# facebookresearch/pytorch3d

Hardware: NVIDIA H100
Metric: rasterize frames/sec (fwd+bwd) 512^2 K=8 (higher is better)
Workload: dtype f32

## Files before the change

### pytorch3d_b200/csrc/raster_meshes.cu

```cuda
#include <cfloat>
#include <climits>

#include "binning.cuh"
#include "bulk_copy.cuh"
#include "common.cuh"
#include "raster_math.cuh"

namespace b200r {

constexpr int SETUP_FACES = 256;
#ifndef B200R_MESH_TILE_H
#define B200R_MESH_TILE_H 16
#endif
constexpr int FTW = 16, FTH = B200R_MESH_TILE_H, FTHREADS = FTW * FTH;
static_assert(FTH == 16 || FTH == 8, "16x16 or 16x8 tiles");
constexpr int CHUNK = FTHREADS;
constexpr int SMEMQ_MAX_K = 32;

__device__ __forceinline__ bool face_is_drawable(const Face& f, bool cull_backfaces) {
  const float zmax = fmaxf(fmaxf(f.z0, f.z1), f.z2), zmin = fminf(fminf(f.z0, f.z1), f.z2);
  if (!(zmax >= 0.0f)) return false;
  if ((double)zmin < kEps) return false;
  const float area = edge_fn(f.x0, f.y0, f.x1, f.y1, f.x2, f.y2);
  if (cull_backfaces && area < 0.0f) return false;
// ... 228 lines not shown
    }
#pragma unroll
    for (int r = 0; r < KMAX; ++r) {
      if (r >= n) break;
#pragma unroll
      for (int i = r & 1; i + 1 < KMAX; i += 2) {
        if (i + 1 < n) {
          const bool sw = key_less(z[i + 1], id[i + 1], z[i], id[i]);
          const float za = z[i], zb = z[i + 1];
          z[i] = sw ? zb : za;
          z[i + 1] = sw ? za : zb;
          const int ia = id[i], ib = id[i + 1];
          id[i] = sw ? ib : ia;
          id[i + 1] = sw ? ia : ib;
          const int sa = slot[i], sb = slot[i + 1];
          slot[i] = sw ? sb : sa;
          slot[i + 1] = sw ? sa : sb;
        }
      }
    }
  }
};

template <int KMAX>
struct RegQueue {
  TopK<KMAX> q;
  float4* pay;
  int K;
  __device__ __forceinline__ void reset() { q.init(); }
  __device__ __forceinline__ bool full() const { return q.size >= K; }
  __device__ __forceinline__ float max_z() const { return q.max_z; }
  __device__ __forceinline__ void offer(const Hit& h, int f) { q.offer(h, f, K, pay); }
  __device__ __forceinline__ bool offer_neighbor(const Hit& h, int f, int nb) { return q.offer_neighbor(h, f, nb, pay); }
};

template <bool NB>
struct SmemQueue {
  float* qz;
  int* qi;
  float* qd;
  int K, size, max_idx;
  float max_zv;
  __device__ __forceinline__ void init(unsigned char* base, int K_, int tid) {
    K = K_;
    qz = reinterpret_cast<float*>(base) + tid;
    qi = reinterpret_cast<int*>(base) + K_ * FTHREADS + tid;
    qd = NB ? reinterpret_cast<float*>(base) + 2 * K_ * FTHREADS + tid : nullptr;
    reset();
  }
  __device__ __forceinline__ void reset() {
    size = 0;
    max_idx = -1;
    max_zv = -1000.0f;
  }
  __device__ __forceinline__ bool full() const { return size >= K; }
  __device__ __forceinline__ float max_z() const { return max_zv; }
  __device__ __forceinline__ void put(int slot, const Hit& h, int f) {
    qz[slot * FTHREADS] = h.z;
    qi[slot * FTHREADS] = f;
    if (NB) qd[slot * FTHREADS] = h.dist;
  }
  __device__ __forceinline__ void offer(const Hit& h, int f) {
    if (size < K) {
      put(size, h, f);
      if (h.z > max_zv) {
        max_zv = h.z;
        max_idx = size;
      }
      ++size;
    } else if (h.z < max_zv) {
      const float evicted = max_zv;
      put(max_idx, h, f);
      max_zv = h.z;
      for (int i = 0; i < K; ++i) {
        const float v = qz[i * FTHREADS];
        if (v > max_zv) {
          max_zv = v;
          max_idx = i;
        }
      }
      if (max_zv == evicted) flag_tie();
    } else if (h.z == max_zv) {
      flag_tie();
    }
  }
  __device__ __forceinline__ bool offer_neighbor(const Hit& h, int f, int nb) {
    int at = -1;
    for (int i = 0; i < size; ++i)
      if (qi[i * FTHREADS] == nb) {
        at = i;
        break;
      }
    if (at < 0) return false;
    if (NB && fabsf(h.dist) < fabsf(qd[at * FTHREADS])) {
      put(at, h, f);
      if (h.z > max_zv) {
        max_zv = h.z;
        max_idx = at;
      }
    }
    return true;
  }
  __device__ __forceinline__ void sort() {
    for (int i = 1; i < size; ++i) {
      const float tz = qz[i * FTHREADS];
      const int ti = qi[i * FTHREADS];
      int j = i - 1;
      while (j >= 0 && key_less(tz, ti, qz[j * FTHREADS], qi[j * FTHREADS])) {
        qz[(j + 1) * FTHREADS] = qz[j * FTHREADS];
        qi[(j + 1) * FTHREADS] = qi[j * FTHREADS];
        --j;
      }
      qz[(j + 1) * FTHREADS] = tz;
      qi[(j + 1) * FTHREADS] = ti;
    }
  }
};

struct __align__(16) FaceChunk {
  float4 box[CHUNK];
  float4 a[CHUNK];
  float4 b[CHUNK];
  float4 c[CHUNK];
};

__device__ __forceinline__ void stage_face(FaceChunk& s, int slot, const float* __restrict__ face_verts,
                                           const int64_t* __restrict__ neighbor, int f, float sqrt_blur,
                                           bool cull_backfaces) {
  const float* v = face_verts + (int64_t)f * 9;
  const Face fc = {__ldg(v + 0), __ldg(v + 1), __ldg(v + 2), __ldg(v + 3), __ldg(v + 4),
                   __ldg(v + 5), __ldg(v + 6), __ldg(v + 7), __ldg(v + 8)};
  float xmin = FLT_MAX, xmax = -FLT_MAX, ymin = FLT_MAX, ymax = -FLT_MAX;
  if (face_is_drawable(fc, cull_backfaces)) face_box(fc, sqrt_blur, xmin, xmax, ymin, ymax);
  s.box[slot] = make_float4(xmin, xmax, ymin, ymax);
  s.a[slot] = make_float4(fc.x0, fc.y0, fc.x1, fc.y1);
  s.b[slot] = make_float4(fc.x2, fc.y2, bary_denominator(fc), __int_as_float(f));
  const int nb = neighbor ? (int)__ldg(neighbor + f) : -1;
  s.c[slot] = make_float4(fc.z0, fc.z1, fc.z2, __int_as_float(nb));
}

template <typename T>
__device__ __forceinline__ void out_store(T* ptr, const T v) {
  __stcs(ptr, v);
}

struct FineParams {
  const float* face_verts;
  const int64_t* neighbor;
  const float4* rec;
  const int64_t* first;
  const int64_t* num;
  const int* tile_offset;
  const int* tile_order;
  int* pairs;
  int64_t capacity;
  int n0;
  int N, H, W, K, TY, TX;
  float rx, ry, blur_radius, sqrt_blur;
  int persp, clip, cull;
  int smem_ints;
  int64_t* pix_to_face;
  float* zbuf;
  float* bary;
  float* dists;
};

__device__ __forceinline__ void thread_pixel(int tile_x, int tile_y, int& xo, int& yo) {
  const int lane = threadIdx.x & 31, w = threadIdx.x >> 5;
  xo = tile_x * TILE + (w & 1) * 8 + (lane & 7);
  yo = tile_y * TILE + (w >> 1) * 4 + (lane >> 3);
}
__device__ __forceinline__ void fthread_pixel(int tile_x, int tile_y, int& xo, int& yo) {
  const int lane = threadIdx.x & 31, w = threadIdx.x >> 5;
  xo = tile_x * FTW + (w & 1) * 8 + (lane & 7);
  yo = tile_y * FTH + (w >> 1) * 4 + (lane >> 3);
}

__device__ __forceinline__ float warp_min(float v) {
#pragma unroll
  for (int d = 16; d > 0; d >>= 1) v = fminf(v, __shfl_xor_sync(0xffffffffu, v, d));
  return v;
}
__device__ __forceinline__ float warp_max(float v) {
#pragma unroll
  for (int d = 16; d > 0; d >>= 1) v = fmaxf(v, __shfl_xor_sync(0xffffffffu, v, d));
  return v;
}

constexpr int ROUND = 64;

struct FineStage {
  float4 a[CHUNK];
  float4 b[CHUNK];
  float4 c[CHUNK];
  union {
    float4 box[CHUNK];
    unsigned mask[CHUNK / 32][FTHREADS];
    int sort_buf[2 * FTHREADS];
    unsigned long long sort_buf64[2 * FTHREADS];
  } u;
  unsigned rng[CHUNK];
  float col[FTW], row[FTH];
  int tie;
  unsigned char tie_lane[FTHREADS];
};

__device__ __forceinline__ void flag_tie() {
#ifndef B200R_EXP_NOWATCH
  extern __shared__ __align__(16) unsigned char smem_raw[];
  reinterpret_cast<FineStage*>(smem_raw)->tie = 1;
  reinterpret_cast<FineStage*>(smem_raw)->tie_lane[threadIdx.x] = 1;
#endif
}

template <int P>
__device__ __forceinline__ void store_pair_run(float4* run, const float4 (&mine)[P], int odd, bool vA, bool vB) {
  constexpr int H = P / 2;
  constexpr int CE = (P + 1) / 2;
  float4 recv[H > 0 ? H : 1];
#pragma unroll
  for (int r = 0; r < H; ++r) {
    const float4 send = odd ? mine[2 * (CE + r) - P] : mine[2 * r + 1];
    recv[r].x = __shfl_xor_sync(0xffffffffu, send.x, 1);
    recv[r].y = __shfl_xor_sync(0xffffffffu, send.y, 1);
    recv[r].z = __shfl_xor_sync(0xffffffffu, send.z, 1);
    recv[r].w = __shfl_xor_sync(0xffffffffu, send.w, 1);
  }
#pragma unroll
  for (int j = 0; j < P; ++j) {
    const float4 ve = 2 * j < P ? mine[2 * j < P ? 2 * j : 0] : recv[j >= CE ? j - CE : 0];
    const float4 vo = 2 * j + 1 < P ? recv[2 * j + 1 < P ? j : 0] : mine[2 * j + 1 >= P ? 2 * j + 1 - P : 0];
    const bool target_a = odd ? (2 * j + 1 < P) : (2 * j < P);
    if (target_a ? vA : vB) out_store(run + 2 * j + odd, odd ? vo : ve);
  }
}

template <int P>
__device__ __forceinline__ void store_pair_split(float4* runA, float4* runB, const float4 (&mine)[P], int odd,
                                                 bool vA, bool vB) {
  static_assert(P % 2 == 0, "an even number of 16-byte pieces per run");
  float4 recv[P / 2];
#pragma unroll
  for (int r = 0; r < P / 2; ++r) {
    const float4 send = odd ? mine[2 * r] : mine[2 * r + 1];
    recv[r].x = __shfl_xor_sync(0xffffffffu, send.x, 1);
    recv[r].y = __shfl_xor_sync(0xffffffffu, send.y, 1);
    recv[r].z = __shfl_xor_sync(0xffffffffu, send.z, 1);
    recv[r].w = __shfl_xor_sync(0xffffffffu, send.w, 1);
  }
#pragma unroll
  for (int r = 0; r < P / 2; ++r)
    if (vA) out_store(runA + 2 * r + odd, odd ? recv[r] : mine[2 * r]);
#pragma unroll
  for (int r = 0; r < P / 2; ++r)
    if (vB) out_store(runB + 2 * r + odd, odd ? mine[2 * r + 1] : recv[r]);
}

template <int KMAX>
__device__ __forceinline__ void write_empty_tile(const FineParams& p, int n, int tile_x, int tile_y) {
  const int tid = threadIdx.x;
  const int x0 = tile_x * FTW, y0 = tile_y * FTH;
  const int K = p.K;
  if ((KMAX == 0 || K == KMAX) && (K % 4) == 0 && x0 + FTW <= p.W && y0 + FTH <= p.H) {
    const float4 m1 = make_float4(-1.f, -1.f, -1.f, -1.f);
    const int KK = KMAX > 0 ? KMAX : K;
    const int SEG_I = FTW * KK / 2;
    const int SEG_F = FTW * KK / 4;
#pragma unroll
    for (int e = tid; e < FTH * SEG_I; e += FTHREADS) {
      const int64_t o = (((int64_t)n * p.H + y0 + e / SEG_I) * p.W + x0) * KK;
      out_store(reinterpret_cast<longlong2*>(p.pix_to_face + o) + e % SEG_I, make_longlong2(-1ll, -1ll));
    }
#pragma unroll
    for (int e = tid; e < FTH * SEG_F; e += FTHREADS) {
      const int64_t o = (((int64_t)n * p.H + y0 + e / SEG_F) * p.W + x0) * KK;
      out_store(reinterpret_cast<float4*>(p.zbuf + o) + e % SEG_F, m1);
      out_store(reinterpret_cast<float4*>(p.dists + o) + e % SEG_F, m1);
    }
#pragma unroll
    for (int e = tid; e < FTH * SEG_F * 3; e += FTHREADS) {
      const int64_t o = (((int64_t)n * p.H + y0 + e / (SEG_F * 3)) * p.W + x0) * KK;
      out_store(reinterpret_cast<float4*>(p.bary + o * 3) + e % (SEG_F * 3), m1);
    }
    return;
  }
  int xo, yo;
  fthread_pixel(tile_x, tile_y, xo, yo);
  if (xo >= p.W || yo >= p.H) return;
  const int64_t o = (((int64_t)n * p.H + yo) * p.W + xo) * K;
  for (int k = 0; k < K; ++k) {
    p.pix_to_face[o + k] = -1ll;
    p.zbuf[o + k] = -1.0f;
    p.dists[o + k] = -1.0f;
    p.bary[(o + k) * 3 + 0] = -1.0f;
    p.bary[(o + k) * 3 + 1] = -1.0f;
    p.bary[(o + k) * 3 + 2] = -1.0f;
  }
}

template <class Q, bool NB>
__device__ __forceinline__ void consider_face(const FineStage& sh, int j, float px, float py, float blur_radius,
                                              bool persp, bool clip, Q& q) {
  const float4 fa = sh.a[j], fb = sh.b[j], fc = sh.c[j];
  const Face f = {fa.x, fa.y, fc.x, fa.z, fa.w, fc.y, fb.x, fb.y, fc.z};
  const int nb = NB ? __float_as_int(fc.w) : -1;
  Hit h;
// ... 103 lines not shown
#define B200R_SCAN_LANES 4
#endif
      constexpr int SL = B200R_SCAN_LANES;
      const int dr = tid & (SL - 1);
      for (int fslot = tid / SL; fslot < nc; fslot += FTHREADS / SL) {
        const unsigned rg = sh.rng[fslot];
        const int c_lo = rg & 255, c_hi = (rg >> 8) & 255, r_lo = (rg >> 16) & 255, r_hi = rg >> 24;
        if (c_lo > c_hi) continue;
        const float4 fa = sh.a[fslot], fb = sh.b[fslot];
        const bool pos = fb.z > 0.0f;
        unsigned* mrow = sh.u.mask[fslot >> 5];
        const unsigned bit = 1u << (fslot & 31);
        const float dx0 = fsub(fb.x, fa.z), dy0 = fsub(fb.y, fa.w);
        const float dx1 = fsub(fa.x, fb.x), dy1 = fsub(fa.y, fb.y);
        const float dx2 = fsub(fa.z, fa.x), dy2 = fsub(fa.w, fa.y);
        for (int r = r_lo + dr; r <= r_hi; r += SL) {
          const float qy = sh.row[r];
          const float t0 = fmul(fsub(qy, fa.w), dx0), t1 = fmul(fsub(qy, fb.y), dx1), t2 = fmul(fsub(qy, fa.y), dx2);
          unsigned* mpix = mrow + (r >> 2) * 64 + (r & 3) * 8;
          for (int c0 = c_lo; c0 <= c_hi; c0 += 4) {
#pragma unroll
            for (int u = 0; u < 4; ++u) {
              const int c = c0 + u;
              if (c <= c_hi) {
                const float qx = sh.col[c];
                const float e0 = ffma(fsub(qx, fa.z), dy0, -t0);
                const float e1 = ffma(fsub(qx, fb.x), dy1, -t1);
                const float e2 = ffma(fsub(qx, fa.x), dy2, -t2);
                const bool ok = pos ? (e0 > 0.0f && e1 > 0.0f && e2 > 0.0f) : (e0 < 0.0f && e1 < 0.0f && e2 < 0.0f);
                if (ok) atomicOr(mpix + (c >> 3) * 32 + (c & 7), bit);
              }
            }
          }
        }
      }
      __syncthreads();
      const float px = sh.col[lc], py = sh.row[lr];
#ifdef B200R_EXP_OLDWALK
      for (int w = 0; w < nwords; ++w) {
        unsigned m = sh.u.mask[w][tid];
        while (m != 0u) {
          const int j = w * 32 + __ffs((int)m) - 1;
          m &= m - 1u;
          consider_face<Q, NB>(sh, j, px, py, blur_radius, persp, clip, q);
        }
      }
#else
      {
        int w = 0;
        unsigned m = sh.u.mask[0][tid];
        for (;;) {
          while (m == 0u && ++w < nwords) m = sh.u.mask[w][tid];
          if (m == 0u) break;
          const int j = w * 32 + __ffs((int)m) - 1;
          m &= m - 1u;
          consider_face<Q, NB>(sh, j, px, py, blur_radius, persp, clip, q);
        }
      }
#endif
      continue;
    }
    const float px = sh.col[lc], py = sh.row[lr];
    const bool cull_depth = (clip || !persp) && (order == ORDER_DEPTH || count >= 512);
    const float fc0 = sh.col[lc & 8], fc1 = sh.col[(lc & 8) + 7], fr0 = sh.row[lr & 12], fr1 = sh.row[(lr & 12) + 3];
    const float cmin = fminf(fc0, fc1), cmax = fmaxf(fc0, fc1), rmin = fminf(fr0, fr1), rmax = fmaxf(fr0, fr1);
    const bool warp_active = __any_sync(0xffffffffu, valid);
    for (int sub = 0; sub < nc; sub += ROUND) {
      if (!warp_active) break;
      unsigned m0 = 0, m1 = 0;
      {
        const bool h0 = sub + lane < nc, h1 = sub + 32 + lane < nc;
        float4 b0 = make_float4(FLT_MAX, -FLT_MAX, FLT_MAX, -FLT_MAX), b1 = b0;
        if (h0) b0 = sh.u.box[sub + lane];
        if (h1) b1 = sh.u.box[sub + 32 + lane];
        bool keep0 = h0, keep1 = h1;
#ifndef B200R_EXP_NOCULL
        if (cull_depth) {
          const float zcut = warp_max(!valid ? -FLT_MAX : (q.full() ? q.max_z() : FLT_MAX));
          if (zcut < FLT_MAX) {
            const float cx = 0.5f * (cmin + cmax), cy = 0.5f * (rmin + rmax);
            const float hx = 0.5f * (cmax - cmin) * (1.0f + 1e-6f), hy = 0.5f * (rmax - rmin) * (1.0f + 1e-6f);
            if (h0) {
              const float4 fc = sh.c[sub + lane];
              if (!NB || __float_as_int(fc.w) == -1)
                keep0 = !(face_depth_lower_bound(sh.a[sub + lane], sh.b[sub + lane], fc, cx, cy, hx, hy, persp, clip) >
                          zcut);
            }
            if (h1) {
              const float4 fc = sh.c[sub + 32 + lane];
              if (!NB || __float_as_int(fc.w) == -1)
                keep1 = !(face_depth_lower_bound(sh.a[sub + 32 + lane], sh.b[sub + 32 + lane], fc, cx, cy, hx, hy,
                                                 persp, clip) > zcut);
            }
            if (!keep0) b0 = make_float4(FLT_MAX, -FLT_MAX, FLT_MAX, -FLT_MAX);
            if (!keep1) b1 = make_float4(FLT_MAX, -FLT_MAX, FLT_MAX, -FLT_MAX);
            if (!__any_sync(0xffffffffu, keep0 || keep1)) continue;
          }
        }
#endif
        const bool all0 =
            __all_sync(0xffffffffu, !keep0 || (cmin >= b0.x && cmax <= b0.y && rmin >= b0.z && rmax <= b0.w));
        const bool all1 =
            __all_sync(0xffffffffu, !keep1 || (cmin >= b1.x && cmax <= b1.y && rmin >= b1.z && rmax <= b1.w));
        if (all0 && all1) {
          m0 = __ballot_sync(0xffffffffu, keep0);
          m1 = __ballot_sync(0xffffffffu, keep1);
        } else {
          float col[8], row[4];
#pragma unroll
          for (int c = 0; c < 8; ++c) col[c] = sh.col[(lc & 8) + c];
#pragma unroll
          for (int r = 0; r < 4; ++r) row[r] = sh.row[(lr & 12) + r];
          if (keep0) m0 = box_pixel_mask(b0, col, row);
          if (keep1) m1 = box_pixel_mask(b1, col, row);
          m0 = warp_transpose_bits(m0, lane);
          if (sub + 32 < nc) m1 = warp_transpose_bits(m1, lane);
        }
      }
      unsigned long long mine = valid ? (((unsigned long long)m1 << 32) | m0) : 0ull;
      while (__any_sync(0xffffffffu, mine != 0ull)) {
        if (mine != 0ull) {
          const int j = sub + __ffsll((long long)mine) - 1;
          mine &= mine - 1ull;
          consider_face<Q, NB>(sh, j, px, py, blur_radius, persp, clip, q);
        }
      }
    }
  }
}

__device__ __forceinline__ bool tile_saw_tie(const FineStage& sh) {
#ifdef B200R_EXP_NOWATCH
  return false;
#else
  return __syncthreads_or(sh.tie) != 0;
#endif
}

struct TileWork {
  int tile_x, tile_y, n, seg_begin, count;
  bool overflow;
};
__device__ __forceinline__ TileWork tile_work(const FineParams& p) {
  pdl_wait();
  TileWork t;
  int i = ((p.n0 + blockIdx.z) * p.TY + blockIdx.y) * p.TX + blockIdx.x;
  if (p.tile_order != nullptr) {
    i = p.tile_order[i];
    t.tile_x = i % p.TX;
    const int r = i / p.TX;
    t.tile_y = r % p.TY;
    t.n = r / p.TY;
  } else {
    t.tile_x = blockIdx.x;
    t.tile_y = blockIdx.y;
    t.n = p.n0 + blockIdx.z;
  }
  t.seg_begin = p.tile_offset[i];
  const int seg_end = p.tile_offset[i + 1];
  t.overflow = (int64_t)seg_end > p.capacity || seg_end == INT_MAX;
  t.count = t.overflow ? (int)p.num[t.n] : seg_end - t.seg_begin;
  return t;
}

template <bool NB, bool SCAN>
__device__ __forceinline__ int first_walk_order(const FineParams& p, const TileWork& t) {
  if (t.overflow || NB) return ORDER_INDEX;
  if (SCAN) return ORDER_ARRIVAL;
#ifndef B200R_EXP_DEPTHORDER
  return ORDER_INDEX;
#else
  const bool bound = p.clip != 0 || p.persp == 0;
  return (bound && 2 * t.count <= p.smem_ints) ? ORDER_DEPTH : ORDER_INDEX;
#endif
}

#ifndef B200R_FINE_CTAS
#define B200R_FINE_CTAS 4
#endif
#ifndef B200R_FINE_SCAN_CTAS
#define B200R_FINE_SCAN_CTAS 3
#endif
#ifndef B200R_SMEMQ_CTAS
#define B200R_SMEMQ_CTAS 3
#endif
#ifndef B200R_SMEMQ_SCAN_CTAS
#define B200R_SMEMQ_SCAN_CTAS 2
#endif

template <int KMAX, bool NB, bool SCAN>
__global__ void __launch_bounds__(FTHREADS, SCAN ? B200R_FINE_SCAN_CTAS : B200R_FINE_CTAS) mesh_fine_kernel(const FineParams p) {
  extern __shared__ __align__(16) unsigned char smem_raw[];
  FineStage& sh = *reinterpret_cast<FineStage*>(smem_raw);
  const int tid = threadIdx.x, lane = tid & 31;
  const TileWork t = tile_work(p);
  const int tile_x = t.tile_x, tile_y = t.tile_y, n = t.n;
  if (t.count == 0) {
    write_empty_tile<KMAX>(p, n, tile_x, tile_y);
    return;
  }
  int xo, yo;
  fthread_pixel(tile_x, tile_y, xo, yo);
  const bool valid = xo < p.W && yo < p.H;
  const int lc = xo - tile_x * FTW, lr = yo - tile_y * FTH;

  RegQueue<KMAX> rq;
  rq.q.init();
  rq.pay = reinterpret_cast<float4*>(smem_raw + sizeof(FineStage)) + tid;
  rq.K = p.K;
  TopK<KMAX>& q = rq.q;
  float4* pay = rq.pay;
  const int K = p.K;
  int order = first_walk_order<NB, SCAN>(p, t);
  bool active = valid;
  int scratch_ints = p.smem_ints;
  for (;;) {
  fine_tile_body<RegQueue<KMAX>, NB, SCAN>(p, sh, rq, tile_x, tile_y, n, t.seg_begin, t.count, t.overflow, order,
                                           active, scratch_ints, lc, lr);
  if (order == ORDER_DEPTH) {
    if (tile_saw_tie(sh)) {
      active = valid && sh.tie_lane[tid] != 0;
      if (active) rq.reset();
      order = ORDER_INDEX;
      scratch_ints = (int)(sizeof(FineStage) / sizeof(int));
      __syncthreads();
      continue;
    }
  }
  bool stored = false;
  int slot[KMAX];
  q.sort(slot);
  const int64_t o = (((int64_t)n * p.H + yo) * p.W + xo) * K;
  if constexpr ((KMAX % 4) == 0) {
   if (K == KMAX) {
    const int odd = lane & 1;
    const bool vA = __shfl_sync(0xffffffffu, (int)valid, lane & ~1) != 0;
    const bool vB = __shfl_sync(0xffffffffu, (int)valid, lane | 1) != 0;
    const int64_t oa = o - (int64_t)odd * KMAX;
    {
      float4 piece[KMAX / 2];
#pragma unroll
      for (int k = 0; k < KMAX; k += 2) {
        const long long i0 = k >= q.size ? -1ll : (long long)q.id[k];
        const long long i1 = k + 1 >= q.size ? -1ll : (long long)q.id[k + 1];
        piece[k / 2] = make_float4(__int_as_float((int)(i0 & 0xffffffffll)), __int_as_float((int)(i0 >> 32)),
                                   __int_as_float((int)(i1 & 0xffffffffll)), __int_as_float((int)(i1 >> 32)));
      }
      store_pair_run<KMAX / 2>(reinterpret_cast<float4*>(p.pix_to_face + oa), piece, odd, vA, vB);
    }
    {
      float4 piece[KMAX / 4];
#pragma unroll
      for (int k0 = 0; k0 < KMAX; k0 += 4)
        piece[k0 / 4] = make_float4(k0 + 0 >= q.size ? -1.0f : q.z[k0 + 0], k0 + 1 >= q.size ? -1.0f : q.z[k0 + 1],
                                    k0 + 2 >= q.size ? -1.0f : q.z[k0 + 2], k0 + 3 >= q.size ? -1.0f : q.z[k0 + 3]);
      store_pair_run<KMAX / 4>(reinterpret_cast<float4*>(p.zbuf + oa), piece, odd, vA, vB);
    }
    {
      float4 piece[KMAX / 4];
#pragma unroll
      for (int k0 = 0; k0 < KMAX; k0 += 4) {
        float d[4];
#pragma unroll
        for (int u = 0; u < 4; ++u) d[u] = k0 + u >= q.size ? -1.0f : pay[slot[k0 + u] * FTHREADS].x;
        piece[k0 / 4] = make_float4(d[0], d[1], d[2], d[3]);
      }
      store_pair_run<KMAX / 4>(reinterpret_cast<float4*>(p.dists + oa), piece, odd, vA, vB);
    }
    {
      float4 piece[3 * KMAX / 4];
#pragma unroll
      for (int k0 = 0; k0 < KMAX; k0 += 4) {
        float4 w[4];
#pragma unroll
        for (int u = 0; u < 4; ++u)
          w[u] = k0 + u >= q.size ? make_float4(-1.f, -1.f, -1.f, -1.f) : pay[slot[k0 + u] * FTHREADS];
        piece[3 * (k0 / 4) + 0] = make_float4(w[0].y, w[0].z, w[0].w, w[1].y);
        piece[3 * (k0 / 4) + 1] = make_float4(w[1].z, w[1].w, w[2].y, w[2].z);
        piece[3 * (k0 / 4) + 2] = make_float4(w[2].w, w[3].y, w[3].z, w[3].w);
      }
      store_pair_run<3 * KMAX / 4>(reinterpret_cast<float4*>(p.bary + oa * 3), piece, odd, vA, vB);
    }
    stored = true;
   }
  }
  if (!stored && valid) {
#pragma unroll
    for (int k = 0; k < KMAX; ++k) {
      if (k < K) {
        const bool e = k >= q.size;
        const float4 w = e ? make_float4(-1.f, -1.f, -1.f, -1.f) : pay[slot[k] * FTHREADS];
        p.pix_to_face[o + k] = e ? -1ll : (long long)q.id[k];
        p.zbuf[o + k] = e ? -1.0f : q.z[k];
        p.dists[o + k] = w.x;
        p.bary[(o + k) * 3 + 0] = w.y;
        p.bary[(o + k) * 3 + 1] = w.z;
        p.bary[(o + k) * 3 + 2] = w.w;
      }
    }
  }
  if (order != ORDER_ARRIVAL || !tile_saw_tie(sh)) return;
  order = ORDER_INDEX;
  rq.reset();
  }
}

__device__ __forceinline__ void recompute_hit(const FineParams& p, int fi, float px, float py, Hit& h) {
  const float4* r = p.rec + (int64_t)fi * 4;
  const float4 fa = __ldg(r + 0), fb = __ldg(r + 1), fc = __ldg(r + 2);
  const Face f = {fa.x, fa.y, fc.x, fa.z, fa.w, fc.y, fb.x, fb.y, fc.z};
  eval_pixel_face<false>(px, py, f, fb.z, p.blur_radius, p.persp != 0, p.clip != 0, false, 0.0f, h);
}

template <bool NB, bool SCAN>
__global__ void __launch_bounds__(FTHREADS, SCAN ? B200R_SMEMQ_SCAN_CTAS : B200R_SMEMQ_CTAS) mesh_fine_smemq_kernel(const FineParams p) {
  extern __shared__ __align__(16) unsigned char smem_raw[];
  FineStage& sh = *reinterpret_cast<FineStage*>(smem_raw);
  const int tid = threadIdx.x, lane = tid & 31;
  const TileWork t = tile_work(p);
  const int tile_x = t.tile_x, tile_y = t.tile_y, n = t.n;
  if (t.count == 0) {
    write_empty_tile<0>(p, n, tile_x, tile_y);
    return;
  }
  int xo, yo;
  fthread_pixel(tile_x, tile_y, xo, yo);
  const bool valid = xo < p.W && yo < p.H;
  const int lc = xo - tile_x * FTW, lr = yo - tile_y * FTH;
  const int K = p.K;

  SmemQueue<NB> q;
  q.init(smem_raw + sizeof(FineStage), K, tid);
  int order = first_walk_order<NB, SCAN>(p, t);
  bool active = valid;
  int scratch_ints = p.smem_ints;
  for (;;) {
  fine_tile_body<SmemQueue<NB>, NB, SCAN>(p, sh, q, tile_x, tile_y, n, t.seg_begin, t.count, t.overflow, order, active,
                                          scratch_ints, lc, lr);
  if (order == ORDER_DEPTH) {
    if (tile_saw_tie(sh)) {
      active = valid && sh.tie_lane[tid] != 0;
      if (active) q.reset();
      order = ORDER_INDEX;
      scratch_ints = (int)(sizeof(FineStage) / sizeof(int));
      __syncthreads();
      continue;
    }
  }
  q.sort();
  const float px = sh.col[lc], py = sh.row[lr];
  const int64_t o = (((int64_t)n * p.H + yo) * p.W + xo) * K;
  if ((K & 7) == 0) {
    const int odd = lane & 1;
    const bool vA = __shfl_sync(0xffffffffu, (int)valid, lane & ~1) != 0;
    const bool vB = __shfl_sync(0xffffffffu, (int)valid, lane | 1) != 0;
    const int64_t oa = o - (int64_t)odd * K, ob = oa + K;
    for (int g = 0; g < K; g += 8) {
      float4 pi[4], pzv[2], pd[2], pb[6];
      float z[8], d[8], b[24];
      int id[8];
#pragma unroll
      for (int u = 0; u < 8; ++u) {
        Hit h = {-1.0f, -1.0f, -1.0f, -1.0f, -1.0f};
        id[u] = -1;
        if (g + u < q.size) {
          id[u] = q.qi[(g + u) * FTHREADS];
          recompute_hit(p, id[u], px, py, h);
        }
        z[u] = h.z;
        d[u] = h.dist;
        b[3 * u + 0] = h.b0;
        b[3 * u + 1] = h.b1;
        b[3 * u + 2] = h.b2;
      }
#pragma unroll
      for (int u = 0; u < 4; ++u)
        pi[u] = make_float4(__int_as_float(id[2 * u]), __int_as_float(id[2 * u] >> 31),
                            __int_as_float(id[2 * u + 1]), __int_as_float(id[2 * u + 1] >> 31));
#pragma unroll
      for (int u = 0; u < 2; ++u) {
        pzv[u] = make_float4(z[4 * u], z[4 * u + 1], z[4 * u + 2], z[4 * u + 3]);
        pd[u] = make_float4(d[4 * u], d[4 * u + 1], d[4 * u + 2], d[4 * u + 3]);
      }
#pragma unroll
      for (int u = 0; u < 6; ++u) pb[u] = make_float4(b[4 * u], b[4 * u + 1], b[4 * u + 2], b[4 * u + 3]);
      store_pair_split<4>(reinterpret_cast<float4*>(p.pix_to_face + oa + g),
                          reinterpret_cast<float4*>(p.pix_to_face + ob + g), pi, odd, vA, vB);
      store_pair_split<2>(reinterpret_cast<float4*>(p.zbuf + oa + g), reinterpret_cast<float4*>(p.zbuf + ob + g), pzv,
                          odd, vA, vB);
      store_pair_split<2>(reinterpret_cast<float4*>(p.dists + oa + g), reinterpret_cast<float4*>(p.dists + ob + g),
                          pd, odd, vA, vB);
      store_pair_split<6>(reinterpret_cast<float4*>(p.bary + (oa + g) * 3),
                          reinterpret_cast<float4*>(p.bary + (ob + g) * 3), pb, odd, vA, vB);
    }
  } else if (valid) {
  for (int k = 0; k < K; ++k) {
    Hit h = {-1.0f, -1.0f, -1.0f, -1.0f, -1.0f};
    long long id = -1;
    if (k < q.size) {
      const int fi = q.qi[k * FTHREADS];
      recompute_hit(p, fi, px, py, h);
      id = fi;
    }
    p.pix_to_face[o + k] = id;
    p.zbuf[o + k] = h.z;
    p.dists[o + k] = h.dist;
    p.bary[(o + k) * 3 + 0] = h.b0;
    p.bary[(o + k) * 3 + 1] = h.b1;
    p.bary[(o + k) * 3 + 2] = h.b2;
  }
  }
  if (order != ORDER_ARRIVAL || !tile_saw_tie(sh)) return;
  order = ORDER_INDEX;
  q.reset();
  }
}

__global__ void __launch_bounds__(FTHREADS) mesh_fine_bigk_kernel(const FineParams p) {
  __shared__ FaceChunk s;
  const int tid = threadIdx.x, lane = tid & 31;
  const int t = blockIdx.x;
  const int n = t / (p.TY * p.TX);
  const int tile_y = (t / p.TX) % p.TY, tile_x = t % p.TX;
  int xo, yo;
  fthread_pixel(tile_x, tile_y, xo, yo);
  const bool valid = xo < p.W && yo < p.H;
  const float px = pix_to_ndc(p.W - 1 - xo, p.W, p.rx);
  const float py = pix_to_ndc(p.H - 1 - yo, p.H, p.ry);
  const float fx_lo = warp_min(valid ? px : FLT_MAX), fx_hi = warp_max(valid ? px : -FLT_MAX);
  const float fy_lo = warp_min(valid ? py : FLT_MAX), fy_hi = warp_max(valid ? py : -FLT_MAX);
  pdl_wait();
  const int seg_begin = p.tile_offset[t], seg_end = p.tile_offset[t + 1];
  const bool overflow = (int64_t)seg_end > p.capacity || seg_end == INT_MAX;
  const int64_t mesh_first = p.first[n];
  const int count = overflow ? (int)p.num[n] : seg_end - seg_begin;
  const bool persp = p.persp != 0, clip = p.clip != 0, cull = p.cull != 0;
  const int K = p.K;

  if (!overflow && count > 1)
    cta_sort_segment<FTHREADS>(p.pairs + seg_begin, count, reinterpret_cast<int*>(&s),
                               (int)(sizeof(FaceChunk) / sizeof(int)));

  float qz[B200R_MAX_K], qd[B200R_MAX_K];
  int qi[B200R_MAX_K];
  int qn = 0, q_max_idx = -1;
  float q_max_z = -1000.0f;

  for (int base = 0; base < count; base += CHUNK) {
    const int nc = min(CHUNK, count - base);
    __syncthreads();
    if (tid < nc) {
      const int f = overflow ? (int)(mesh_first + base + tid) : p.pairs[seg_begin + base + tid];
      stage_face(s, tid, p.face_verts, p.neighbor, f, p.sqrt_blur, cull);
// ... 131 lines not shown
                                             float (&out)[9]) {
  const float* v = p.face_verts + fi * 9;
  const Face f = {__ldg(v + 0), __ldg(v + 1), __ldg(v + 2), __ldg(v + 3), __ldg(v + 4),
                  __ldg(v + 5), __ldg(v + 6), __ldg(v + 7), __ldg(v + 8)};
  const float den = bary_denominator(f);
  float w0, w1, w2;
  bary_coords(px, py, f, den, w0, w1, w2);
  float c0 = w0, c1 = w1, c2 = w2;
  if (persp) bary_persp(c0, c1, c2, f.z0, f.z1, f.z2);
  float k0 = c0, k1 = c1, k2 = c2;
  if (clip) bary_clip(k0, k1, k2);
  const bool inside = c0 > 0.0f && c1 > 0.0f && c2 > 0.0f;
  const float sgd = inside ? -gd : gd;

  float2 dv0 = make_float2(0.f, 0.f), dv1 = dv0, dv2 = dv0;
  {
    const float e01 = point_line_dist(px, py, f.x0, f.y0, f.x1, f.y1);
    const float e02 = point_line_dist(px, py, f.x0, f.y0, f.x2, f.y2);
    const float e12 = point_line_dist(px, py, f.x1, f.y1, f.x2, f.y2);
    if (e01 <= e02 && e01 <= e12)
      point_line_bwd(px, py, f.x0, f.y0, f.x1, f.y1, sgd, dv0, dv1);
    else if (e02 <= e01 && e02 <= e12)
      point_line_bwd(px, py, f.x0, f.y0, f.x2, f.y2, sgd, dv0, dv2);
    else if (e12 <= e01 && e12 <= e02)
      point_line_bwd(px, py, f.x1, f.y1, f.x2, f.y2, sgd, dv1, dv2);
  }

  float g0 = gb0 + gz * f.z0, g1 = gb1 + gz * f.z1, g2 = gb2 + gz * f.z2;
  if (clip) {
    const float m0 = fmaxf(c0, 0.0f), m1 = fmaxf(c1, 0.0f), m2 = fmaxf(c2, 0.0f);
    float sum = m0 + m1 + m2, gsc = 1.0f;
    if (sum < 1e-5f) {
      gsc = 0.0f;
      sum = 1e-5f;
    }
    const float inv = __frcp_rn(sum), inv2 = gsc * inv * inv;
    const float s0 = -m0 * inv2, s1 = -m1 * inv2, s2 = -m2 * inv2;
    const float cross = g0 * s0 + g1 * s1 + g2 * s2;
    const float n0 = c0 < 0.0f ? 0.0f : g0 * inv + cross;
    const float n1 = c1 < 0.0f ? 0.0f : g1 * inv + cross;
    const float n2 = c2 < 0.0f ? 0.0f : g2 * inv + cross;
    g0 = n0;
    g1 = n1;
    g2 = n2;
  }
  float dz0 = 0.0f, dz1 = 0.0f, dz2 = 0.0f;
  if (persp) {
    const float t0 = w0 * f.z1 * f.z2, t1 = f.z0 * w1 * f.z2, t2 = f.z0 * f.z1 * w2;
    const float dn = fmaxf(t0 + t1 + t2, 1e-8f);
    const float rdn = __frcp_rn(dn);
    const float gdn = (-t0 * g0 - t1 * g1 - t2 * g2) * rdn * rdn;
    const float h0 = gdn + g0 * rdn, h1 = gdn + g1 * rdn, h2 = gdn + g2 * rdn;
    g0 = h0 * f.z1 * f.z2;
    g1 = h1 * f.z0 * f.z2;
    g2 = h2 * f.z0 * f.z1;
    dz0 = h1 * w1 * f.z2 + h2 * w2 * f.z1;
    dz1 = h0 * w0 * f.z2 + h2 * w2 * f.z0;
    dz2 = h0 * w0 * f.z1 + h1 * w1 * f.z0;
  }
  float2 bv0 = make_float2(0.f, 0.f), bv1 = bv0, bv2 = bv0;
  {
    const float rden = __frcp_rn(den);
    const float e0 = edge_fn(px, py, f.x1, f.y1, f.x2, f.y2);
    const float e1 = edge_fn(px, py, f.x2, f.y2, f.x0, f.y0);
    const float e2 = edge_fn(px, py, f.x0, f.y0, f.x1, f.y1);
    float2 dp, da, db, ap, aa, ab;
    const float garea = -(g0 * e0 + g1 * e1 + g2 * e2) * rden * rden;
    edge_bwd(f.x2, f.y2, f.x0, f.y0, f.x1, f.y1, garea, ap, aa, ab);
    bv2.x += ap.x; bv2.y += ap.y;
    bv0.x += aa.x; bv0.y += aa.y;
    bv1.x += ab.x; bv1.y += ab.y;
    edge_bwd(px, py, f.x1, f.y1, f.x2, f.y2, g0 * rden, dp, da, db);
    bv1.x += da.x; bv1.y += da.y;
    bv2.x += db.x; bv2.y += db.y;
    edge_bwd(px, py, f.x2, f.y2, f.x0, f.y0, g1 * rden, dp, da, db);
    bv2.x += da.x; bv2.y += da.y;
    bv0.x += db.x; bv0.y += db.y;
    edge_bwd(px, py, f.x0, f.y0, f.x1, f.y1, g2 * rden, dp, da, db);
    bv0.x += da.x; bv0.y += da.y;
    bv1.x += db.x; bv1.y += db.y;
  }
  out[0] = bv0.x + dv0.x;
  out[1] = bv0.y + dv0.y;
  out[2] = gz * k0 + dz0;
  out[3] = bv1.x + dv1.x;
  out[4] = bv1.y + dv1.y;
  out[5] = gz * k1 + dz1;
  out[6] = bv2.x + dv2.x;
  out[7] = bv2.y + dv2.y;
  out[8] = gz * k2 + dz2;
}

__device__ __forceinline__ void red_add_v2(float* addr, float a, float b) {
  asm volatile("red.global.add.v2.f32 [%0], {%1, %2};" ::"l"(addr), "f"(a), "f"(b) : "memory");
}
__device__ __forceinline__ void warp_scatter(const BackwardParams& p, int face, float (&g)[9], int lane) {
  const unsigned grp = __match_any_sync(0xffffffffu, face);
  const unsigned above = lane == 31 ? 0u : grp & (0xffffffffu << (lane + 1));
  int next = (face >= 0 && above != 0u) ? __ffs((int)above) - 1 : -1;
  while (__any_sync(0xffffffffu, next >= 0)) {
    const int src = next >= 0 ? next : lane;
#pragma unroll
    for (int i = 0; i < 9; ++i) {
      const float v = __shfl_sync(0xffffffffu, g[i], src);
      if (next >= 0) g[i] += v;
    }
    const int nn = __shfl_sync(0xffffffffu, next, src);
    next = next >= 0 ? nn : -1;
  }
  if (face >= 0 && lane == __ffs((int)grp) - 1) {
    if (p.faces != nullptr) {
      const int64_t* fc = p.faces + (int64_t)face * 3;
#pragma unroll
      for (int j = 0; j < 3; ++j) {
        const int64_t vi = __ldg(fc + j);
        if (vi < 0 || vi >= p.V) continue;
        float* o = p.grad_verts + vi * 3;
#ifndef B200R_EXP_BWD_SCALAR_RED
        if (p.g_vec) {
          const bool odd = (vi & 1) != 0;
          const float s1 = odd ? g[3 * j] : g[3 * j + 2];
          const float a = odd ? g[3 * j + 1] : g[3 * j], b = odd ? g[3 * j + 2] : g[3 * j + 1];
          if (s1 != 0.0f) atomicAdd(o + (odd ? 0 : 2), s1);
          if (a != 0.0f || b != 0.0f) red_add_v2(o + (odd ? 1 : 0), a, b);
          continue;
        }
#endif
#pragma unroll
        for (int c = 0; c < 3; ++c)
          if (g[3 * j + c] != 0.0f) atomicAdd(o + c, g[3 * j + c]);
      }
    } else {
      float* o = p.grad_face_verts + (int64_t)face * 9;
#ifndef B200R_EXP_BWD_SCALAR_RED
      if (p.g_vec) {
        const int odd = face & 1;
        atomicAdd(o + (odd ? 0 : 8), odd ? g[0] : g[8]);
#pragma unroll
        for (int j = 0; j < 4; ++j)
          red_add_v2(o + 2 * j + odd, odd ? g[2 * j + 1] : g[2 * j], odd ? g[2 * j + 2] : g[2 * j + 1]);
        return;
      }
#endif
#pragma unroll
      for (int i = 0; i < 9; ++i) atomicAdd(o + i, g[i]);
    }
  }
}

#ifndef B200R_BWD_PF_CTAS
#define B200R_BWD_PF_CTAS 3
#endif
#ifndef B200R_BWD_CTAS
#define B200R_BWD_CTAS 4
#endif
template <int GV, bool PF>
__global__ void __launch_bounds__(TILE_THREADS, PF ? B200R_BWD_PF_CTAS : B200R_BWD_CTAS) mesh_backward_kernel(const BackwardParams p) {
  const int lane = threadIdx.x & 31;
  const int tile_x = blockIdx.x, tile_y = blockIdx.y, n = p.n0 + blockIdx.z;
  int xo, yo;
  thread_pixel(tile_x, tile_y, xo, yo);
  const bool in_image = xo < p.W && yo < p.H;
  const float px = pix_to_ndc(p.W - 1 - xo, p.W, p.rx);
  const float py = pix_to_ndc(p.H - 1 - yo, p.H, p.ry);
  const int K = p.K;
  const int64_t o = in_image ? (((int64_t)n * p.H + yo) * p.W + xo) * K : 0;
  const bool persp = p.persp != 0, clip = p.clip != 0;
  constexpr int G = GV > 0 ? GV : 1;
  static_assert(!PF || GV == 8, "the prefetching variant is the K % 8 == 0 kernel");

  for (int k0 = 0; k0 < K; k0 += G) {
    int fk[G];
    if (GV > 0) {
#pragma unroll
      for (int k = 0; k < G; k += 2) {
        longlong2 v = make_longlong2(-1, -1);
        if (in_image) v = __ldg(reinterpret_cast<const longlong2*>(p.pix_to_face + o + k0 + k));
        fk[k] = (int)v.x;
        fk[k + 1] = (int)v.y;
      }
    } else {
      fk[0] = in_image ? (int)p.pix_to_face[o + k0] : -1;
    }
    float pz[PF ? 4 : 1], pd[PF ? 4 : 1], pb[PF ? 12 : 1];
    if (PF) {
      float4 vz = make_float4(0.f, 0.f, 0.f, 0.f), vd = vz, b0 = vz, b1 = vz, b2 = vz;
      if (fk[0] >= 0) {
        vz = __ldg(reinterpret_cast<const float4*>(p.grad_zbuf + o + k0));
        vd = __ldg(reinterpret_cast<const float4*>(p.grad_dists + o + k0));
        const float4* gb = reinterpret_cast<const float4*>(p.grad_bary + (o + k0) * 3);
        b0 = __ldg(gb + 0);
        b1 = __ldg(gb + 1);
        b2 = __ldg(gb + 2);
      }
      pz[0] = vz.x; pz[1] = vz.y; pz[2] = vz.z; pz[3] = vz.w;
      pd[0] = vd.x; pd[1] = vd.y; pd[2] = vd.z; pd[3] = vd.w;
      pb[0] = b0.x; pb[1] = b0.y; pb[2] = b0.z; pb[3] = b0.w;
      pb[4] = b1.x; pb[5] = b1.y; pb[6] = b1.z; pb[7] = b1.w;
      pb[8] = b2.x; pb[9] = b2.y; pb[10] = b2.z; pb[11] = b2.w;
    }
#pragma unroll 1
    for (int j = 0; j < G; ++j) {
      const int face = fk[0];
#pragma unroll
      for (int u = 0; u + 1 < G; ++u) fk[u] = fk[u + 1];
      float gz = 0.f, gd = 0.f, gb0 = 0.f, gb1 = 0.f, gb2 = 0.f;
      if (PF) {
        gz = pz[0]; gd = pd[0]; gb0 = pb[0]; gb1 = pb[1]; gb2 = pb[2];
#pragma unroll
        for (int u = 0; u < 3; ++u) {
          pz[u] = pz[u + 1];
          pd[u] = pd[u + 1];
        }
#pragma unroll
        for (int u = 0; u < 9; ++u) pb[u] = pb[u + 3];
      }
      if (!__any_sync(0xffffffffu, face >= 0)) continue;
      float g[9] = {0.f, 0.f, 0.f, 0.f, 0.f, 0.f, 0.f, 0.f, 0.f};
      if (face >= 0) {
        const int64_t i = o + k0 + j;
        if (!PF || j >= 4) {
          gz = __ldg(p.grad_zbuf + i);
          gd = __ldg(p.grad_dists + i);
          gb0 = __ldg(p.grad_bary + i * 3);
          gb1 = __ldg(p.grad_bary + i * 3 + 1);
          gb2 = __ldg(p.grad_bary + i * 3 + 2);
        }
        backward_one(p, px, py, face, gz, gd, gb0, gb1, gb2, persp, clip, g);
      }
      warp_scatter(p, face, g, lane);
    }
  }
}

}

__global__ void __launch_bounds__(256) mesh_gather_kernel(const float* __restrict__ verts, int64_t V,
                                                          const int64_t* __restrict__ faces, int64_t F,
                                                          float* __restrict__ face_verts_out) {
  const int64_t e = (int64_t)blockIdx.x * blockDim.x + threadIdx.x;
  if (e >= F * 3) return;
  const int64_t vi = __ldg(faces + e);
  const bool ok = vi >= 0 && vi < V;
#pragma unroll
  for (int c = 0; c < 3; ++c) face_verts_out[e * 3 + c] = ok ? __ldg(verts + vi * 3 + c) : __int_as_float(0x7fc00000);
}

using namespace b200r;

extern "C" size_t b200r_rasterize_meshes_workspace_bytes(int64_t F, int32_t N, int32_t H, int32_t W,
                                                         int64_t pair_capacity) {
  if (F < 0 || N < 0 || H < 0 || W < 0) return 0;
  return carve_workspace(nullptr, F, N, H, W, pair_capacity, FTH, FTW).bytes +
         FACE_RECORD_BYTES * (size_t)(F > 0 ? F : 1);
}

static int forward_impl(const float* face_verts, const float* verts, int64_t V, const int64_t* faces,
                        float* face_verts_out, int64_t F, const int64_t* first, const int64_t* num,
                        const int64_t* neighbor, int32_t N, int32_t H, int32_t W, float blur_radius, int32_t K,
                        int32_t perspective_correct, int32_t clip_barycentric_coords, int32_t cull_backfaces,
                        int64_t* pix_to_face, float* zbuf, float* bary, float* dists, void* workspace,
                        size_t workspace_bytes, int64_t pair_capacity, void* stream_) {
  cudaStream_t stream = static_cast<cudaStream_t>(stream_);
  if (K > B200R_MAX_K) return fail(B200R_ERR_INVALID_ARGUMENT, "Must have points_per_pixel <= 150");
  if (F < 0 || N < 0 || H < 0 || W < 0 || K < 0) return fail(B200R_ERR_INVALID_ARGUMENT, "negative size");
  if (F > INT_MAX) return fail(B200R_ERR_INVALID_ARGUMENT, "more than 2^31-1 packed faces are not supported");
  if ((int64_t)N * H * W * K == 0) return B200R_OK;
  const int TY = div_up(H, FTH), TX = div_up(W, FTW);
  if (TY > 0xFFFE || TX > 0xFFFE) return fail(B200R_ERR_INVALID_ARGUMENT, "image too large");
  const int64_t ntiles = (int64_t)N * TY * TX;
  if (ntiles > INT_MAX) return fail(B200R_ERR_INVALID_ARGUMENT, "too many tiles");
  BinWorkspace ws = carve_workspace(workspace, F, N, H, W, pair_capacity, FTH, FTW);
  const size_t nrec = (size_t)(F > 0 ? F : 1);
  if (workspace == nullptr || workspace_bytes < ws.bytes + FACE_RECORD_BYTES * nrec)
    return fail(B200R_ERR_WORKSPACE, "workspace too small for rasterize_meshes_forward");
  float4* rec = reinterpret_cast<float4*>(static_cast<char*>(workspace) + ws.bytes);

  const float rx = ndc_range(W, H), ry = ndc_range(H, W);
  const float sqrt_blur = sqrtf(blur_radius);

  const bool prof = profiling_enabled();
  if (prof) phase_timer().record(0, stream);
#ifndef B200R_EXP_MEMSET_NODE
  zero_ints_kernel<<<(unsigned)((ntiles + 1023) / 1024), 256, 0, stream>>>(ws.tile_count, ntiles);
  B200R_LAUNCHED("zero_ints_kernel");
#else
  B200R_CUDA_OK(cudaMemsetAsync(ws.tile_count, 0, sizeof(int) * (size_t)ntiles, stream));
#endif
  if (F > 0) {
    const unsigned sgrid = (unsigned)((F + SETUP_FACES - 1) / SETUP_FACES);
#ifndef B200R_EXP_MEMSET_NODE
#define B200R_SETUP_LAUNCH(KERNEL, ...) B200R_CUDA_OK(launch_chained(KERNEL, dim3(sgrid), dim3(SETUP_FACES), 0, stream, __VA_ARGS__))
#else
#define B200R_SETUP_LAUNCH(KERNEL, ...) KERNEL<<<sgrid, SETUP_FACES, 0, stream>>>(__VA_ARGS__)
#endif
    if (faces != nullptr) {
      B200R_SETUP_LAUNCH(mesh_setup_count_kernel<true>, (const float*)nullptr, verts, V, faces, face_verts_out, neighbor, F,
                         first, num, N, H, W, TY, TX, rx, ry, sqrt_blur, cull_backfaces, ws.rect, ws.tile_count, rec);
      face_verts = face_verts_out;
    } else {
      B200R_SETUP_LAUNCH(mesh_setup_count_kernel<false>, face_verts, (const float*)nullptr, (int64_t)0,
                         (const int64_t*)nullptr, (float*)nullptr, neighbor, F, first, num, N, H, W, TY, TX, rx, ry,
                         sqrt_blur, cull_backfaces, ws.rect, ws.tile_count, rec);
    }
#undef B200R_SETUP_LAUNCH
    B200R_LAUNCHED("mesh_setup_count_kernel");
  }
#ifdef B200R_EXP_NOTILEORDER
  int* const tile_order = nullptr;
#else
  int* const tile_order = (blur_radius > 0.0f && ntiles < (1ll << ORDER_BITS)) ? ws.tile_order : nullptr;
#endif
  B200R_CUDA_OK(launch_chained(tile_scan_kernel, dim3(1), dim3(1024), 0, stream, ws.tile_count, ws.tile_offset,
                               (int)ntiles, tile_order));
  B200R_LAUNCHED("tile_scan_kernel");
  if (F > 0) {
    B200R_CUDA_OK(launch_chained(tile_fill_kernel<true>, dim3((unsigned)((F + 255) / 256)), dim3(256), 0, stream,
                                 ws.rect, F, TY, TX, ws.tile_count, ws.pairs, ws.capacity));
    B200R_LAUNCHED("tile_fill_kernel");
  }
  if (prof) phase_timer().record(1, stream);
  FineParams p;
  p.face_verts = face_verts;
  p.neighbor = neighbor;
  p.rec = rec;
  p.n0 = 0;
  p.first = first;
  p.num = num;
  p.tile_offset = ws.tile_offset;
  p.tile_order = tile_order;
  p.pairs = ws.pairs;
  p.capacity = ws.capacity;
  p.N = N; p.H = H; p.W = W; p.K = K; p.TY = TY; p.TX = TX;
  p.rx = rx; p.ry = ry; p.blur_radius = blur_radius; p.sqrt_blur = sqrt_blur;
  p.persp = perspective_correct; p.clip = clip_barycentric_coords; p.cull = cull_backfaces;
  p.smem_ints = 0;
  p.pix_to_face = pix_to_face; p.zbuf = zbuf; p.bary = bary; p.dists = dists;
  const unsigned grid = (unsigned)ntiles;
  const bool no_blur = !(blur_radius > 0.0f);
  int dev_ = 0;
  B200R_CUDA_OK(cudaGetDevice(&dev_));
#define B200R_FINE_LAUNCH(KERNEL, SMEM_MAX, SMEM)                                                         \
  do {                                                                                                   \
    static bool configured[64] = {};                                                                     \
    if (dev_ < 0 || dev_ >= 64 || !configured[dev_]) {                                                   \
      B200R_CUDA_OK(cudaFuncSetAttribute(KERNEL, cudaFuncAttributeMaxDynamicSharedMemorySize, (int)(SMEM_MAX))); \
      if (dev_ >= 0 && dev_ < 64) configured[dev_] = true;                                               \
    }                                                                                                    \
    p.smem_ints = (int)((SMEM) / sizeof(int));                                                           \
    for (p.n0 = 0; p.n0 < N; p.n0 += 65535) {                                                            \
      const dim3 grid3((unsigned)TX, (unsigned)TY, (unsigned)min(N - p.n0, 65535));                      \
      B200R_CUDA_OK(launch_chained(KERNEL, grid3, dim3(FTHREADS), (SMEM), stream, p));                   \
    }                                                                                                    \
  } while (0)
#define B200R_FINE(KM)                                                                                    \
  do {                                                                                                   \
    constexpr size_t smem_ = sizeof(FineStage) + sizeof(float4) * KM * FTHREADS;                         \
    if (neighbor && no_blur)                                                                             \
      B200R_FINE_LAUNCH((mesh_fine_kernel<KM, true, true>), smem_, smem_);                               \
    else if (neighbor)                                                                                   \
      B200R_FINE_LAUNCH((mesh_fine_kernel<KM, true, false>), smem_, smem_);                              \
    else if (no_blur)                                                                                    \
      B200R_FINE_LAUNCH((mesh_fine_kernel<KM, false, true>), smem_, smem_);                              \
    else                                                                                                 \
      B200R_FINE_LAUNCH((mesh_fine_kernel<KM, false, false>), smem_, smem_);                             \
  } while (0)
  if (K <= 1)
    B200R_FINE(1);
  else if (K <= 2)
    B200R_FINE(2);
  else if (K <= 4)
    B200R_FINE(4);
  else if (K <= 8)
    B200R_FINE(8);
  else if (K <= SMEMQ_MAX_K) {
    const size_t smem_max_nb = sizeof(FineStage) + (size_t)SMEMQ_MAX_K * FTHREADS * 12;
    const size_t smem_max = sizeof(FineStage) + (size_t)SMEMQ_MAX_K * FTHREADS * 8;
    const size_t smem_nb = sizeof(FineStage) + (size_t)K * FTHREADS * 12;
    const size_t smem = sizeof(FineStage) + (size_t)K * FTHREADS * 8;
    if (neighbor && no_blur)
      B200R_FINE_LAUNCH((mesh_fine_smemq_kernel<true, true>), smem_max_nb, smem_nb);
    else if (neighbor)
      B200R_FINE_LAUNCH((mesh_fine_smemq_kernel<true, false>), smem_max_nb, smem_nb);
    else if (no_blur)
      B200R_FINE_LAUNCH((mesh_fine_smemq_kernel<false, true>), smem_max, smem);
    else
      B200R_FINE_LAUNCH((mesh_fine_smemq_kernel<false, false>), smem_max, smem);
  } else
    B200R_CUDA_OK(launch_chained(mesh_fine_bigk_kernel, dim3(grid), dim3(FTHREADS), 0, stream, p));
#undef B200R_FINE
#undef B200R_FINE_LAUNCH
  B200R_LAUNCHED("mesh_fine_kernel");
  if (prof) {
    phase_timer().record(2, stream);
    phase_timer().have_fwd = true;
  }
  return B200R_OK;
}

extern "C" int b200r_rasterize_meshes_forward(const float* face_verts, int64_t F, const int64_t* first,
                                              const int64_t* num, const int64_t* neighbor, int32_t N, int32_t H,
                                              int32_t W, float blur_radius, int32_t K, int32_t bin_size,
                                              int32_t max_faces_per_bin, int32_t perspective_correct,
                                              int32_t clip_barycentric_coords, int32_t cull_backfaces,
                                              int64_t* pix_to_face, float* zbuf, float* bary, float* dists,
                                              void* workspace, size_t workspace_bytes, int64_t pair_capacity,
                                              void* stream_) {
  (void)bin_size;
  (void)max_faces_per_bin;
  return forward_impl(face_verts, nullptr, 0, nullptr, nullptr, F, first, num, neighbor, N, H, W, blur_radius, K,
                      perspective_correct, clip_barycentric_coords, cull_backfaces, pix_to_face, zbuf, bary, dists,
                      workspace, workspace_bytes, pair_capacity, stream_);
}

extern "C" int b200r_rasterize_meshes_forward_indexed(const float* verts, int64_t V, const int64_t* faces, int64_t F,
                                                      const int64_t* first, const int64_t* num,
                                                      const int64_t* neighbor, int32_t N, int32_t H, int32_t W,
                                                      float blur_radius, int32_t K, int32_t perspective_correct,
                                                      int32_t clip_barycentric_coords, int32_t cull_backfaces,
                                                      int64_t* pix_to_face, float* zbuf, float* bary, float* dists,
                                                      float* face_verts_out, void* workspace,
                                                      size_t workspace_bytes, int64_t pair_capacity,
                                                      void* stream_) {
  if (V < 0) return fail(B200R_ERR_INVALID_ARGUMENT, "negative size");
  if (F > 0 && (faces == nullptr || face_verts_out == nullptr || (V > 0 && verts == nullptr)))
    return fail(B200R_ERR_INVALID_ARGUMENT, "verts, faces and face_verts_out must not be null");
  if ((int64_t)N * H * W * K == 0 && F > 0) {
    cudaStream_t stream = static_cast<cudaStream_t>(stream_);
    mesh_gather_kernel<<<(unsigned)((F * 3 + 255) / 256), 256, 0, stream>>>(verts, V, faces, F, face_verts_out);
    B200R_LAUNCHED("mesh_gather_kernel");
    return B200R_OK;
  }
  return forward_impl(nullptr, verts, V, F > 0 ? faces : nullptr, face_verts_out, F, first, num, neighbor, N, H, W,
                      blur_radius, K, perspective_correct, clip_barycentric_coords, cull_backfaces, pix_to_face,
                      zbuf, bary, dists, workspace, workspace_bytes, pair_capacity, stream_);
}

static int backward_impl(const float* face_verts, int64_t F, const int64_t* pix_to_face, const float* grad_zbuf,
                         const float* grad_bary, const float* grad_dists, int32_t N, int32_t H, int32_t W, int32_t K,
                         int32_t perspective_correct, int32_t clip_barycentric_coords, float* grad_face_verts,
                         const int64_t* faces, float* grad_verts, int64_t V, void* stream_) {
  cudaStream_t stream = static_cast<cudaStream_t>(stream_);
  if (F < 0 || N < 0 || H < 0 || W < 0 || K < 0) return fail(B200R_ERR_INVALID_ARGUMENT, "negative size");
  if (F == 0) return B200R_OK;
  if (faces == nullptr) B200R_CUDA_OK(cudaMemsetAsync(grad_face_verts, 0, sizeof(float) * 9 * (size_t)F, stream));
  if ((int64_t)N * H * W * K == 0) return B200R_OK;
  const int TY = div_up(H, TILE), TX = div_up(W, TILE);
  BackwardParams p;
  p.face_verts = face_verts; p.pix_to_face = pix_to_face;
  p.grad_zbuf = grad_zbuf; p.grad_bary = grad_bary; p.grad_dists = grad_dists;
  p.N = N; p.H = H; p.W = W; p.K = K; p.TY = TY; p.TX = TX;
  p.F = F;
  p.g_vec = (reinterpret_cast<uintptr_t>(faces != nullptr ? grad_verts : grad_face_verts) & 7u) == 0 ? 1 : 0;
  p.rx = ndc_range(W, H); p.ry = ndc_range(H, W);
  p.persp = perspective_correct; p.clip = clip_barycentric_coords;
  p.grad_face_verts = grad_face_verts;
  p.faces = faces;
  p.grad_verts = grad_verts;
  p.V = V;
  const bool prof = profiling_enabled();
  if (prof) phase_timer().record(3, stream);
  for (p.n0 = 0; p.n0 < N; p.n0 += 65535) {
    const dim3 bgrid((unsigned)TX, (unsigned)TY, (unsigned)min(N - p.n0, 65535));
    const bool aligned = ((reinterpret_cast<uintptr_t>(grad_zbuf) | reinterpret_cast<uintptr_t>(grad_bary) |
                           reinterpret_cast<uintptr_t>(grad_dists)) & 15u) == 0;
#ifdef B200R_EXP_BWDPF
    const bool prefetch = aligned;
#else
    const bool prefetch = false && aligned;
#endif
    if ((K & 7) == 0 && prefetch)
      mesh_backward_kernel<8, true><<<bgrid, TILE_THREADS, 0, stream>>>(p);
    else if ((K & 7) == 0)
      mesh_backward_kernel<8, false><<<bgrid, TILE_THREADS, 0, stream>>>(p);
    else if ((K & 3) == 0)
      mesh_backward_kernel<4, false><<<bgrid, TILE_THREADS, 0, stream>>>(p);
    else
      mesh_backward_kernel<0, false><<<bgrid, TILE_THREADS, 0, stream>>>(p);
  }
  B200R_LAUNCHED("mesh_backward_kernel");
  if (prof) {
    phase_timer().record(4, stream);
    phase_timer().have_bwd = true;
// ... 29 lines not shown
```

Before: 18330.

## Scatter fine-raster tile order with golden-ratio coprime stride; lower backward CTA bound

When no explicit tile order is given, the fine kernel now maps each block index to a tile through a multiplicative permutation whose stride is near the golden ratio times the tile count and coprime to it. The aim is to spread heavy and light tiles evenly across SMs, so that neighbouring blocks do not all land on the same busy screen region. The change also lowers the backward kernel's minimum-CTAs launch bound from 4 to 3, giving it more registers per thread. It adds debug-only macros that skip stores or treat every tile as empty, and it costs a 64-bit modulo per block plus less contiguous output writes.

```diff
diff --git a/pytorch3d_b200/csrc/raster_meshes.cu b/pytorch3d_b200/csrc/raster_meshes.cu
--- a/pytorch3d_b200/csrc/raster_meshes.cu
+++ b/pytorch3d_b200/csrc/raster_meshes.cu
@@ -404,6 +404,7 @@
   const int64_t* num;
   const int* tile_offset;
   const int* tile_order;
+  int64_t tile_stride;
   int* pairs;
   int64_t capacity;
   int n0;
@@ -813,9 +814,11 @@
     t.tile_y = r % p.TY;
     t.n = r / p.TY;
   } else {
-    t.tile_x = blockIdx.x;
-    t.tile_y = blockIdx.y;
-    t.n = p.n0 + blockIdx.z;
+    i = (int)(i * p.tile_stride % ((int64_t)p.N * p.TY * p.TX));
+    t.tile_x = i % p.TX;
+    const int r = i / p.TX;
+    t.tile_y = r % p.TY;
+    t.n = r / p.TY;
   }
   t.seg_begin = p.tile_offset[i];
   const int seg_end = p.tile_offset[i + 1];
@@ -856,8 +859,14 @@
   const int tid = threadIdx.x, lane = tid & 31;
   const TileWork t = tile_work(p);
   const int tile_x = t.tile_x, tile_y = t.tile_y, n = t.n;
+#ifdef B200R_EXP_FINE_ALLEMPTY
+  if (true) {
+#else
   if (t.count == 0) {
+#endif
+#ifndef B200R_EXP_FINE_NOSTORE
     write_empty_tile<KMAX>(p, n, tile_x, tile_y);
+#endif
     return;
   }
   int xo, yo;
@@ -888,9 +897,17 @@
       continue;
     }
   }
-  bool stored = false;
   int slot[KMAX];
   q.sort(slot);
+#ifdef B200R_EXP_FINE_NOSTORE
+  {
+    float s = 0.0f;
+#pragma unroll
+    for (int k = 0; k < KMAX; ++k) s += q.z[k] + (float)q.id[k] + pay[slot[k] * FTHREADS].x;
+    if (__float_as_int(s) == 0x7fbadbad) p.zbuf[0] = s;
+  }
+#else
+  bool stored = false;
   const int64_t o = (((int64_t)n * p.H + yo) * p.W + xo) * K;
   if constexpr ((KMAX % 4) == 0) {
    if (K == KMAX) {
@@ -960,6 +977,7 @@
       }
     }
   }
+#endif
   if (order != ORDER_ARRIVAL || !tile_saw_tie(sh)) return;
   order = ORDER_INDEX;
   rq.reset();
@@ -1397,7 +1415,7 @@
 #define B200R_BWD_PF_CTAS 3
 #endif
 #ifndef B200R_BWD_CTAS
-#define B200R_BWD_CTAS 4
+#define B200R_BWD_CTAS 3
 #endif
 template <int GV, bool PF>
 __global__ void __launch_bounds__(TILE_THREADS, PF ? B200R_BWD_PF_CTAS : B200R_BWD_CTAS) mesh_backward_kernel(const BackwardParams p) {
@@ -1498,6 +1516,20 @@
   if (F < 0 || N < 0 || H < 0 || W < 0) return 0;
   return carve_workspace(nullptr, F, N, H, W, pair_capacity, FTH, FTW).bytes +
          FACE_RECORD_BYTES * (size_t)(F > 0 ? F : 1);
+}
+
+static int64_t fine_tile_stride(int64_t ntiles) {
+  int64_t s = (int64_t)((double)ntiles * 0.6180339887498949);
+  if (s < 1) s = 1;
+  for (;; ++s) {
+    int64_t a = ntiles, b = s;
+    while (b != 0) {
+      const int64_t t = a % b;
+      a = b;
+      b = t;
+    }
+    if (a == 1) return s;
+  }
 }
 
 static int forward_impl(const float* face_verts, const float* verts, int64_t V, const int64_t* faces,
@@ -1574,6 +1606,7 @@
   p.num = num;
   p.tile_offset = ws.tile_offset;
   p.tile_order = tile_order;
+  p.tile_stride = fine_tile_stride(ntiles);
   p.pairs = ws.pairs;
   p.capacity = ws.capacity;
   p.N = N; p.H = H; p.W = W; p.K = K; p.TY = TY; p.TX = TX;
```

Measured after the change: 18570 (median of 6 runs). 1.01x the previous value.
